# marlbenchmark/off-policy

Measured on NVIDIA H100. Metric: learner grad-steps/sec, higher is better.
Workload: dtype f32

## Files before the change

off-policy_b200/csrc/agent_bwd.cu:

```cuda
#include "mx_internal.h"
#include "mx_kernels.h"
#include "mx_tile.cuh"

static inline size_t qhead_bwd_smem(int A, int APL) { return (size_t)(A * MX_H * 9 + 8 * 32 * APL + 2 * 8 * MX_H + 2 * MX_H) * sizeof(float); }

template <int APL>
__global__ void __launch_bounds__(256) k_qhead_bwd(QHeadBwdArgs a) {
  constexpr int AR = 32 * APL;
  MX_DYN_SMEM(smem);
  const int tid = threadIdx.x, lane = tid & 31, warp = tid >> 5;
  const int A = a.A, AW = A * MX_H;
  float* wq_s = smem;
  float* dw_w = wq_s + AW;
  float* db_w = dw_w + 8 * AW;
  float* dg_w = db_w + 8 * AR;
  float* dbt_w = dg_w + 8 * MX_H;
  float* lg_s = dbt_w + 8 * MX_H;
  float* lb_s = lg_s + MX_H;
  for (int i = tid; i < AW; i += blockDim.x) wq_s[i] = a.theta[a.wq + i];
  for (int i = tid; i < 8 * AW + 8 * AR; i += blockDim.x) dw_w[i] = 0.f;
  for (int i = tid; i < MX_H; i += blockDim.x) { lg_s[i] = a.theta[a.lno_g + i]; lb_s[i] = a.theta[a.lno_b + i]; }
  MX_PDL_WAIT();
  __syncthreads();
  const int wglobal = blockIdx.x * (blockDim.x >> 5) + warp;
  const int wtotal = gridDim.x * (blockDim.x >> 5);
  const int T1 = a.T + 1, N = a.N;
  float dg0 = 0.f, dg1 = 0.f, db0 = 0.f, db1 = 0.f;
  float* my_dw = dw_w + warp * AW;
  for (int m = wglobal; m < a.M; m += wtotal) {
    const int n = m % N;
    const int bt = m / N;
    const int t = bt % T1, b = bt / T1;
    float* out = a.dh_out + (size_t)m * MX_H;
    if (t >= a.T) {
      out[lane] = 0.f; out[lane + 32] = 0.f;
      continue;
    }
    const size_t e = (size_t)b * a.T + t;
    const int act = a.act_idx[(size_t)b * a.ld_tn + (size_t)t * N + n];
    const float dqv = a.dq_taken[e * N + n];
    const float* h = a.hall + (size_t)m * MX_H;
    const float mean = a.sto[2 * (size_t)m], rstd = a.sto[2 * (size_t)m + 1];
    const float xh0 = (h[lane] - mean) * rstd, xh1 = (h[lane + 32] - mean) * rstd;
    const float y0 = xh0 * lg_s[lane] + lb_s[lane], y1 = xh1 * lg_s[lane + 32] + lb_s[lane + 32];
    const float dy0 = dqv * wq_s[act * MX_H + lane], dy1 = dqv * wq_s[act * MX_H + lane + 32];
    my_dw[act * MX_H + lane] += dqv * y0;
    my_dw[act * MX_H + lane + 32] += dqv * y1;
    if (lane == 0) db_w[warp * AR + act] += dqv;
    dg0 += dy0 * xh0; dg1 += dy1 * xh1; db0 += dy0; db1 += dy1;
    const float dx0 = dy0 * lg_s[lane], dx1 = dy1 * lg_s[lane + 32];
    const float c1 = mx_warp_sum(dx0 + dx1) * (1.f / MX_H);
    const float c2 = mx_warp_sum(dx0 * xh0 + dx1 * xh1) * (1.f / MX_H);
    out[lane] = rstd * (dx0 - c1 - xh0 * c2);
    out[lane + 32] = rstd * (dx1 - c1 - xh1 * c2);
  }
  dg_w[warp * MX_H + lane] = dg0; dg_w[warp * MX_H + lane + 32] = dg1;
  dbt_w[warp * MX_H + lane] = db0; dbt_w[warp * MX_H + lane + 32] = db1;
  __syncthreads();
  float* gp = a.gpart + (size_t)blockIdx.x * a.P;
  for (int i = tid; i < AW; i += blockDim.x) {
    float v = 0.f;
#pragma unroll
    for (int w = 0; w < 8; ++w) v += dw_w[w * AW + i];
    gp[a.wq + i] = v;
  }
  for (int i = tid; i < A; i += blockDim.x) {
    float v = 0.f;
#pragma unroll
    for (int w = 0; w < 8; ++w) v += db_w[w * AR + i];
    gp[a.bq + i] = v;
  }
  for (int i = tid; i < MX_H; i += blockDim.x) {
    float g = 0.f, bb = 0.f;
#pragma unroll
    for (int w = 0; w < 8; ++w) { g += dg_w[w * MX_H + i]; bb += dbt_w[w * MX_H + i]; }
    gp[a.lno_g + i] = g; gp[a.lno_b + i] = bb;
  }
}

#define BWD_THREADS 256

template <int RPC>
__global__ void __launch_bounds__(BWD_THREADS, 1) k_gru_bwd(GruBwdArgs a) {
  constexpr int RING = RPC <= 2 ? 8 : 4;
  constexpr int PF = RING - 2;
  __shared__ __align__(16) float ops_s[RING][RPC][6][MX_H];
  __shared__ __align__(16) float dgh_s[2][RPC][MX_G];
  const int tid = threadIdx.x;
  const int k = tid >> 2, s = tid & 3;
  const int row0 = blockIdx.x * RPC;
  float2 w[24];
#pragma unroll
  for (int m = 0; m < 12; ++m)
#pragma unroll
    for (int c = 0; c < 2; ++c) {
      const int j = 16 * m + 4 * s + 2 * c;
      w[2 * m + c] = make_float2(a.theta[a.whh + j * MX_H + k], a.theta[a.whh + (j + 1) * MX_H + k]);
    }
  const int T1 = a.T1 > 0 ? a.T1 : a.T + 1, N = a.N;
  MX_PDL_WAIT();

  constexpr int NPIECE = (RPC * 96 + BWD_THREADS - 1) / BWD_THREADS;
  const float* pf_src[NPIECE];
  size_t pf_stride[NPIECE];
  int pf_dst[NPIECE];
  bool pf_hprev[NPIECE];
  const float* pf_h0[NPIECE];
  const int t_first = a.T - 1;
#pragma unroll
  for (int u = 0; u < NPIECE; ++u) {
    const int c = tid + u * BWD_THREADS;
    pf_dst[u] = -1; pf_src[u] = a.hall; pf_stride[u] = 0; pf_hprev[u] = false; pf_h0[u] = nullptr;
    if (c < RPC * 96) {
      const int r = c / 96, rem = c % 96, op = rem / 16, q4 = rem % 16;
      const int row = row0 + r;
      if (row < a.R) {
        pf_dst[u] = (r * 6 + op) * MX_H + 4 * q4;
        const size_t m0 = ((size_t)(row / N) * T1) * N + (row % N);
        const float* base;
        if (op < 3) { base = a.gates + m0 * MX_G + op * MX_H + 4 * q4; pf_stride[u] = (size_t)N * MX_G; }
        else if (op == 3) { base = a.hn + m0 * MX_H + 4 * q4; pf_stride[u] = (size_t)N * MX_H; }
        else if (op == 4) { base = a.hall + m0 * MX_H + 4 * q4; pf_stride[u] = (size_t)N * MX_H; pf_hprev[u] = true;
                            if (a.h0) pf_h0[u] = a.h0 + (size_t)row * MX_H + 4 * q4; }
        else { base = a.dh_out + m0 * MX_H + 4 * q4; pf_stride[u] = (size_t)N * MX_H; }
        pf_src[u] = base + (ptrdiff_t)(pf_hprev[u] ? t_first - 1 : t_first) * (ptrdiff_t)pf_stride[u];
      }
    }
  }
  auto prefetch = [&](int t) {
    if (t >= 0) {
#pragma unroll
      for (int u = 0; u < NPIECE; ++u) {
        if (pf_dst[u] >= 0) {
          float* dst = &ops_s[t & (RING - 1)][0][0][0] + pf_dst[u];
          const bool first = pf_hprev[u] && t == 0;
          mx_cp16z(dst, first ? (pf_h0[u] ? pf_h0[u] : a.hall) : pf_src[u], (first && !pf_h0[u]) ? 0 : 16);
          pf_src[u] -= pf_stride[u];
        }
      }
    }
    mx_cp_commit();
  };

  for (int idx = tid; idx < RING * RPC * 6 * MX_H; idx += BWD_THREADS) (&ops_s[0][0][0][0])[idx] = 0.f;
  for (int tz = a.T; tz < T1; ++tz)
    for (int idx = tid; idx < RPC * MX_G; idx += BWD_THREADS) {
      const int r = idx / MX_G, c = idx % MX_G;
      const int row = row0 + r;
      if (row < a.R) {
        const size_t mm = (((size_t)(row / N) * T1) + tz) * N + (row % N);
        a.dgi[mm * MX_G + c] = 0.f;
      }
    }
  float* dgp[RPC];
  bool dg_on[RPC];
  float carry[RPC];
  const size_t dg_stride = (size_t)N * MX_G;
  const int sq = s < 3 ? s : 2;
#pragma unroll
  for (int r = 0; r < RPC; ++r) {
    const int row = row0 + r;
    const bool valid = row < a.R;
    const size_t m0 = valid ? ((size_t)(row / N) * T1) * N + (row % N) : 0;
    dgp[r] = a.dgi + (m0 + (size_t)t_first * N) * MX_G + sq * MX_H + k;
    dg_on[r] = valid && s < 3;
    carry[r] = 0.f;
  }
  __syncthreads();
#pragma unroll
  for (int d = 0; d < PF; ++d) prefetch(t_first - d);
  mx_cp_wait<PF - 1>();
  __syncthreads();

  auto step = [&](const int t, const int cur) {
    prefetch(t - PF);
    const float* os = &ops_s[t & (RING - 1)][0][0][0];
    float cz[RPC];
#pragma unroll
    for (int r = 0; r < RPC; ++r) {
      const float* o = os + r * 6 * MX_H;
      const float rg = o[k], zg = o[MX_H + k], ng = o[2 * MX_H + k], hn = o[3 * MX_H + k], hp = o[4 * MX_H + k];
      const float dh = o[5 * MX_H + k] + carry[r];
      const float d_n = dh * (1.f - zg) * (1.f - ng * ng);
      const float d_z = dh * (hp - ng) * zg * (1.f - zg);
      const float d_r = d_n * hn * rg * (1.f - rg);
      const float vg = s == 0 ? d_r : (s == 1 ? d_z : d_n);
      const float vs = s == 0 ? d_r : (s == 1 ? d_z : d_n * rg);
      dgh_s[cur][r][sq * MX_H + k] = vs;
      if (dg_on[r]) *dgp[r] = vg;
      dgp[r] -= dg_stride;
      cz[r] = dh * zg;
    }
    mx_cp_wait<PF - 1>();
    __syncthreads();
#pragma unroll
    for (int r = 0; r < RPC; ++r) {
      float2 p0 = make_float2(0.f, 0.f), p1 = p0, p2 = p0;
#pragma unroll
      for (int m = 0; m < 12; m += 3) {
        const float4 d0 = mx_ld4(&dgh_s[cur][r][16 * m + 4 * s]);
        const float4 d1 = mx_ld4(&dgh_s[cur][r][16 * (m + 1) + 4 * s]);
        const float4 d2 = mx_ld4(&dgh_s[cur][r][16 * (m + 2) + 4 * s]);
        p0 = mx_ffma2(w[2 * m], make_float2(d0.x, d0.y), p0); p0 = mx_ffma2(w[2 * m + 1], make_float2(d0.z, d0.w), p0);
        p1 = mx_ffma2(w[2 * m + 2], make_float2(d1.x, d1.y), p1); p1 = mx_ffma2(w[2 * m + 3], make_float2(d1.z, d1.w), p1);
        p2 = mx_ffma2(w[2 * m + 4], make_float2(d2.x, d2.y), p2); p2 = mx_ffma2(w[2 * m + 5], make_float2(d2.z, d2.w), p2);
      }
      p0 = mx_fadd2(mx_fadd2(p0, p1), p2);
      float p = p0.x + p0.y;
      p += __shfl_xor_sync(0xffffffffu, p, 1);
      p += __shfl_xor_sync(0xffffffffu, p, 2);
      carry[r] = cz[r] + p;
    }
  };
  int t = t_first;
  for (; t >= 1; t -= 2) { step(t, 0); step(t - 1, 1); }
  if (t == 0) step(0, 0);
  mx_cp_wait<0>();
}

#define BWD2_THREADS 128
template <int ROWS>
__global__ void __launch_bounds__(BWD2_THREADS, 2) k_gru_bwd2(GruBwdArgs a) {
  constexpr int RING = 8, PF = 6;
  __shared__ __align__(16) float ops_s[RING][ROWS][6][MX_H];
  __shared__ __align__(16) float dgh_s[2][ROWS][MX_G];
  const int tid = threadIdx.x;
  const int kp = tid >> 2, s = tid & 3;
  float2 w0[24], w1[24];
#pragma unroll
  for (int m = 0; m < 12; ++m)
#pragma unroll
    for (int c = 0; c < 2; ++c) {
      const int j = 16 * m + 4 * s + 2 * c;
      w0[2 * m + c] = make_float2(a.theta[a.whh + j * MX_H + 2 * kp], a.theta[a.whh + (j + 1) * MX_H + 2 * kp]);
      w1[2 * m + c] = make_float2(a.theta[a.whh + j * MX_H + 2 * kp + 1], a.theta[a.whh + (j + 1) * MX_H + 2 * kp + 1]);
    }
  const int T1 = a.T1 > 0 ? a.T1 : a.T + 1, N = a.N;
  MX_PDL_WAIT();
  const int t_first = a.T - 1;
  const bool pf_on = tid < 96;
  const int op = pf_on ? tid / 16 : 0, q4 = tid % 16;
  const bool pf_hprev = op == 4;
  const size_t pf_stride = (size_t)N * (op < 3 ? MX_G : MX_H);
  const int ku = 2 * kp + (s & 1);
  const int half = s >> 1;
  const size_t dg_stride = (size_t)N * MX_G;
  bool rok[ROWS];
  const float* pf_src[ROWS];
  const float* pf_h0[ROWS];
  float* dgp[ROWS];
  float carry[ROWS];
#pragma unroll
  for (int r = 0; r < ROWS; ++r) {
    const int row = blockIdx.x * ROWS + r;
    rok[r] = row < a.R;
    const int rr = rok[r] ? row : 0;
    const size_t m0 = ((size_t)(rr / N) * T1) * N + (rr % N);
    const float* base = op < 3 ? a.gates + m0 * MX_G + op * MX_H + 4 * q4 : (op == 3 ? a.hn : (op == 4 ? a.hall : a.dh_out)) + m0 * MX_H + 4 * q4;
    pf_src[r] = base + (ptrdiff_t)(pf_hprev ? t_first - 1 : t_first) * (ptrdiff_t)pf_stride;
    pf_h0[r] = (pf_hprev && a.h0) ? a.h0 + (size_t)rr * MX_H + 4 * q4 : nullptr;
    if (rok[r])
      for (int tz = a.T; tz < T1; ++tz)
        for (int c = tid; c < MX_G; c += BWD2_THREADS) a.dgi[(m0 + (size_t)tz * N) * MX_G + c] = 0.f;
    dgp[r] = a.dgi + (m0 + (size_t)t_first * N) * MX_G + ku;
    carry[r] = 0.f;
  }
  float* pf_dst = &ops_s[0][0][op][4 * q4];
  auto prefetch = [&](int t) {
    if (t >= 0 && pf_on) {
      const bool first = pf_hprev && t == 0;
#pragma unroll
      for (int r = 0; r < ROWS; ++r) {
        if (rok[r]) mx_cp16z(pf_dst + ((t & (RING - 1)) * ROWS + r) * (6 * MX_H), first ? (pf_h0[r] ? pf_h0[r] : a.hall) : pf_src[r], (first && !pf_h0[r]) ? 0 : 16);
        pf_src[r] -= pf_stride;
      }
    }
    mx_cp_commit();
  };
  if (ROWS > 1) {
    for (int idx = tid; idx < RING * ROWS * 6 * MX_H; idx += BWD2_THREADS) (&ops_s[0][0][0][0])[idx] = 0.f;
    __syncthreads();
  }
#pragma unroll
  for (int d = 0; d < PF; ++d) prefetch(t_first - d);
  mx_cp_wait<PF - 1>();
  __syncthreads();

  auto step = [&](const int t, const int cur) {
    prefetch(t - PF);
    float cz[ROWS];
#pragma unroll
    for (int r = 0; r < ROWS; ++r) {
      const float* o = &ops_s[t & (RING - 1)][r][0][0];
      const float rg = o[ku], zg = o[MX_H + ku], ng = o[2 * MX_H + ku], hn = o[3 * MX_H + ku], hp = o[4 * MX_H + ku];
      const float dh = o[5 * MX_H + ku] + carry[r];
      const float d_n = dh * (1.f - zg) * (1.f - ng * ng);
      const float d_z = dh * (hp - ng) * zg * (1.f - zg);
      const float d_r = d_n * hn * rg * (1.f - rg);
      dgh_s[cur][r][(half ? 2 * MX_H : 0) + ku] = half ? d_n * rg : d_r;
      if (!half) dgh_s[cur][r][MX_H + ku] = d_z;
      if (rok[r]) {
        dgp[r][half ? 2 * MX_H : 0] = half ? d_n : d_r;
        if (!half) dgp[r][MX_H] = d_z;
      }
      dgp[r] -= dg_stride;
      cz[r] = dh * zg;
    }
    mx_cp_wait<PF - 1>();
    __syncthreads();
#pragma unroll
    for (int r = 0; r < ROWS; ++r) {
      float2 a0 = make_float2(0.f, 0.f), a1 = a0, b0 = a0, b1 = a0;
#pragma unroll
      for (int m = 0; m < 12; ++m) {
        const float4 d = mx_ld4(&dgh_s[cur][r][16 * m + 4 * s]);
        const float2 lo = make_float2(d.x, d.y), hi = make_float2(d.z, d.w);
        a0 = mx_ffma2(w0[2 * m], lo, a0); b0 = mx_ffma2(w1[2 * m], lo, b0);
        a1 = mx_ffma2(w0[2 * m + 1], hi, a1); b1 = mx_ffma2(w1[2 * m + 1], hi, b1);
      }
      a0 = mx_fadd2(a0, a1); b0 = mx_fadd2(b0, b1);
      float p0 = a0.x + a0.y, p1 = b0.x + b0.y;
      p0 += __shfl_xor_sync(0xffffffffu, p0, 1); p1 += __shfl_xor_sync(0xffffffffu, p1, 1);
      p0 += __shfl_xor_sync(0xffffffffu, p0, 2); p1 += __shfl_xor_sync(0xffffffffu, p1, 2);
      carry[r] = cz[r] + ((s & 1) ? p1 : p0);
    }
  };
  int t = t_first;
  for (; t >= 1; t -= 2) { step(t, 0); step(t - 1, 1); }
  if (t == 0) step(0, 0);
  mx_cp_wait<0>();
}

struct FrontBwdSmem {
  int ldi, ld64, ldg;
  int o_dgi, o_dgn, o_x, o_hp, o_u, o_da, o_x0, o_xh0, o_dx0, o_wc, o_col, o_stat, o_lnp, total;
};
static FrontBwdSmem front_bwd_smem(int in_dim, int TM, bool gru_ext = false) {
  FrontBwdSmem s;
  const int I64 = mx_round_up(in_dim, 64);
  s.ldi = mx_ld(I64); s.ld64 = mx_ld(64); s.ldg = mx_ld(MX_G);
  int o = 0;
  s.o_dgi = o; o += TM * s.ldg;
  s.o_dgn = o; o += gru_ext ? 0 : TM * s.ld64;
  s.o_x = o; o += TM * s.ld64;
  s.o_hp = o; o += gru_ext ? 0 : TM * s.ld64;
  s.o_u = o; o += TM * s.ld64;
  s.o_da = o; o += TM * s.ld64;
  s.o_x0 = o; o += TM * s.ldi;
  s.o_xh0 = o; o += TM * s.ldi;
  s.o_dx0 = o; o += TM * s.ldi;
  s.o_wc = o; o += 64 * s.ld64;
  s.o_col = o; o += 2 * I64 + 4 * 64;
  s.o_stat = o; o += 3 * TM * 2;
  s.o_lnp = o; o += 4 * 64;
  s.total = o;
  return s;
}

template <int RM>
MX_DEVINL void ln64_bwd_relu(bool act_tanh, float (&v)[RM][4], const float* u_s, int ld, const float* stat , const float* gamma_s,
                             float (&dg)[4], float (&db)[4]) {
  const int tx = threadIdx.x & 15, ty = threadIdx.x >> 4;
#pragma unroll
  for (int i = 0; i < RM; ++i) {
    const int r = ty * RM + i;
    const float mean = stat[2 * r], rstd = stat[2 * r + 1];
    const float4 u4 = mx_ld4(u_s + r * ld + 4 * tx);
    const float uu[4] = {u4.x, u4.y, u4.z, u4.w};
    float xh[4], dx[4], s1 = 0.f, s2 = 0.f;
#pragma unroll
    for (int j = 0; j < 4; ++j) {
      xh[j] = (uu[j] - mean) * rstd;
      dg[j] = fmaf(v[i][j], xh[j], dg[j]);
      db[j] += v[i][j];
      dx[j] = v[i][j] * gamma_s[4 * tx + j];
      s1 += dx[j]; s2 += dx[j] * xh[j];
    }
    s1 = mx_row16_sum(s1) * (1.f / 64.f);
    s2 = mx_row16_sum(s2) * (1.f / 64.f);
#pragma unroll
    for (int j = 0; j < 4; ++j) {
      const float du = rstd * (dx[j] - s1 - xh[j] * s2);
      v[i][j] = act_tanh ? du * (1.f - uu[j] * uu[j]) : (uu[j] > 0.f ? du : 0.f);
    }
  }
}

template <int RM>
__global__ void __launch_bounds__(MX_TILE_THREADS) k_front_bwd(FrontBwdArgs a, FrontBwdSmem sm) {
  constexpr int TM = 16 * RM;
  MX_DYN_SMEM(smem);
  const MxNetLayout L = a.L;
  const float* __restrict__ th = a.theta;
  const int I = L.in_dim, I64 = mx_round_up(I, 64);
  float* dgi_s = smem + sm.o_dgi; float* dgn_s = smem + sm.o_dgn; float* x_s = smem + sm.o_x; float* hp_s = smem + sm.o_hp;
  float* u_s = smem + sm.o_u; float* da_s = smem + sm.o_da; float* x0_s = smem + sm.o_x0; float* xh0_s = smem + sm.o_xh0;
  float* Wc = smem + sm.o_wc;
  float* col0g = smem + sm.o_col; float* col0b = col0g + I64;
  float* col1g = col0b + I64; float* col1b = col1g + 64;
  float* col2g = col1b + 64; float* col2b = col2g + 64;
  float* st0_s = smem + sm.o_stat; float* st1_s = st0_s + 2 * TM; float* st2_s = st1_s + 2 * TM;
  float* ln1g_s = smem + sm.o_lnp; float* ln1b_s = ln1g_s + 64; float* ln2g_s = ln1b_s + 64; float* ln2b_s = ln2g_s + 64;
  const int tid = threadIdx.x, tx = tid & 15, ty = tid >> 4;
  const int ntiles = (a.M + TM - 1) / TM;
  const int T1 = a.T1 > 0 ? a.T1 : a.T + 1, N = a.N;
  const bool ldx_vec = (a.ldx & 3) == 0;
  const bool wg = !a.skip_wgrad;
  const bool wgemm = wg && !a.wgrad_external;
  const bool gru_here = !a.gru_wgrad_ext;
  float* dx0_s = smem + sm.o_dx0;
  float* gp = a.gpart + (size_t)blockIdx.x * a.P;
  for (int i = tid; i < 2 * I64 + 4 * 64; i += MX_TILE_THREADS) col0g[i] = 0.f;
  if (tid < 64) { ln1g_s[tid] = th[L.ln1_g + tid]; ln1b_s[tid] = th[L.ln1_b + tid]; ln2g_s[tid] = th[L.ln2_g + tid]; ln2b_s[tid] = th[L.ln2_b + tid]; }
  float dg1[4] = {0.f, 0.f, 0.f, 0.f}, db1[4] = {0.f, 0.f, 0.f, 0.f}, dg2[4] = {0.f, 0.f, 0.f, 0.f}, db2[4] = {0.f, 0.f, 0.f, 0.f};
  int iter = 0;
  MX_PDL_WAIT();
  for (int tile = blockIdx.x; tile < ntiles; tile += gridDim.x, ++iter) {
    const int m0 = tile * TM;
    const bool accum = iter > 0;
    __syncthreads();
    mx_stage_rows(dgi_s, sm.ldg, a.dgi, MX_G, m0, a.M, TM, MX_G);
    if (!gru_here) {}
    else if (!a.no_gru) mx_stage_rows(x_s, sm.ld64, a.gates, MX_G, m0, a.M, TM, MX_H);
    else for (int i = tid; i < TM * sm.ld64; i += MX_TILE_THREADS) x_s[i] = 0.f;
    mx_stage_rows(u_s, sm.ld64, a.u2, MX_H, m0, a.M, TM, MX_H);
    for (int r = tid >> 4; gru_here && r < TM; r += MX_TILE_THREADS / 16) {
      const int m = m0 + r;
      const bool has = !a.no_gru && m < a.M && ((m / N) % T1) > 0;
      float* d = hp_s + r * sm.ld64 + 4 * tx;
      if (has) mx_cp16(d, a.hall + (size_t)(m - N) * MX_H + 4 * tx);
      else if (m < a.M && a.h0) mx_cp16(d, a.h0 + (size_t)m * MX_H + 4 * tx);
      else mx_st4(d, make_float4(0.f, 0.f, 0.f, 0.f));
    }
    if (ldx_vec) mx_stage_rows(x0_s, sm.ldi, a.X, a.ldx, m0, a.M, TM, mx_round_up(I, 4));
    mx_cp_commit();
    for (int i = tid; i < 3 * TM * 2; i += MX_TILE_THREADS) {
      const int which = i / (2 * TM), rr = (i % (2 * TM)) >> 1, comp = i & 1;
      const int m = m0 + rr;
      const float* src = which == 0 ? a.st0 : (which == 1 ? a.st1 : a.st2);
      st0_s[i] = (m < a.M && (which > 0 || a.feature_norm)) ? src[2 * (size_t)m + comp] : 0.f;
    }
    mx_cp_wait<0>();
    __syncthreads();
    for (int idx = tid; gru_here && idx < TM * MX_H; idx += MX_TILE_THREADS) {
      const int r = idx >> 6, c = idx & 63;
      const int o = r * sm.ld64 + c;
      dgn_s[o] = dgi_s[r * sm.ldg + 2 * MX_H + c] * x_s[o];
      x_s[o] = (m0 + r < a.M) ? (u_s[o] - st2_s[2 * r]) * st2_s[2 * r + 1] * ln2g_s[c] + ln2b_s[c] : 0.f;
    }
    __syncthreads();
    if (wgemm && gru_here) {
      for (int nb = 0; nb < 3; ++nb) {
        mx_wgrad_block(dgi_s + nb * 64, sm.ldg, x_s, sm.ld64, TM, gp + L.wih, MX_G, MX_H, nb * 64, 0, accum);
        if (a.no_gru) continue;
        const float* dgh = nb < 2 ? dgi_s + nb * 64 : dgn_s;
        const int ldd = nb < 2 ? sm.ldg : sm.ld64;
        mx_wgrad_block(dgh, ldd, hp_s, sm.ld64, TM, gp + L.whh + nb * 64 * MX_H, 64, MX_H, 0, 0, accum);
      }
      mx_colsum(dgi_s, sm.ldg, TM, MX_G, gp + L.bih, accum);
      if (!a.no_gru) {
        mx_colsum(dgi_s, sm.ldg, TM, 2 * MX_H, gp + L.bhh, accum);
        mx_colsum(dgn_s, sm.ld64, TM, MX_H, gp + L.bhh + 2 * MX_H, accum);
      }
    }
    float v[RM][4];
#pragma unroll
    for (int i = 0; i < RM; ++i)
#pragma unroll
      for (int jx = 0; jx < 4; ++jx) v[i][jx] = 0.f;
    for (int nc = 0; nc < 3; ++nc) {
      __syncthreads();
      mx_stage_weight(Wc, sm.ld64, th + L.wih, MX_G, MX_H, MX_H, nc * 64, 0, 64);
      __syncthreads();
      mx_mm_nn<RM>(dgi_s + nc * 64, sm.ldg, Wc, sm.ld64, v);
    }
    ln64_bwd_relu<RM>(a.act_tanh != 0, v, u_s, sm.ld64, st2_s, ln2g_s, dg2, db2);
    __syncthreads();
#pragma unroll
    for (int i = 0; i < RM; ++i) mx_st4(da_s + (ty * RM + i) * sm.ld64 + 4 * tx, make_float4(v[i][0], v[i][1], v[i][2], v[i][3]));
    if (a.wgrad_external) {
#pragma unroll
      for (int i = 0; i < RM; ++i) {
        const int m = m0 + ty * RM + i;
        if (m < a.M) mx_st4(a.da2_out + (size_t)m * MX_H + 4 * tx, make_float4(v[i][0], v[i][1], v[i][2], v[i][3]));
      }
    }
    mx_stage_rows(u_s, sm.ld64, a.u1, MX_H, m0, a.M, TM, MX_H);
    mx_cp_commit();
    mx_cp_wait<0>();
    __syncthreads();
    for (int idx = tid; idx < TM * MX_H; idx += MX_TILE_THREADS) {
      const int r = idx >> 6, c = idx & 63;
      const int o = r * sm.ld64 + c;
      x_s[o] = (m0 + r < a.M) ? (u_s[o] - st1_s[2 * r]) * st1_s[2 * r + 1] * ln1g_s[c] + ln1b_s[c] : 0.f;
    }
    __syncthreads();
    if (wgemm) {
      mx_wgrad_block(da_s, sm.ld64, x_s, sm.ld64, TM, gp + L.w2, MX_H, MX_H, 0, 0, accum);
      mx_colsum(da_s, sm.ld64, TM, MX_H, gp + L.b2, accum);
    }
    mx_stage_weight(Wc, sm.ld64, th + L.w2, MX_H, MX_H, MX_H, 0, 0, 64);
    __syncthreads();
#pragma unroll
    for (int i = 0; i < RM; ++i)
#pragma unroll
      for (int jx = 0; jx < 4; ++jx) v[i][jx] = 0.f;
    mx_mm_nn<RM>(da_s, sm.ld64, Wc, sm.ld64, v);
    ln64_bwd_relu<RM>(a.act_tanh != 0, v, u_s, sm.ld64, st1_s, ln1g_s, dg1, db1);
    __syncthreads();
#pragma unroll
    for (int i = 0; i < RM; ++i) mx_st4(da_s + (ty * RM + i) * sm.ld64 + 4 * tx, make_float4(v[i][0], v[i][1], v[i][2], v[i][3]));
    if (a.wgrad_external) {
#pragma unroll
      for (int i = 0; i < RM; ++i) {
        const int m = m0 + ty * RM + i;
        if (m < a.M) mx_st4(a.da1_out + (size_t)m * MX_H + 4 * tx, make_float4(v[i][0], v[i][1], v[i][2], v[i][3]));
      }
    }
    for (int idx = tid; idx < TM * I64; idx += MX_TILE_THREADS) {
      const int r = idx / I64, c = idx - r * I64, m = m0 + r;
      float xh = 0.f, x0 = 0.f;
      if (m < a.M && c < I) {
        const float x = ldx_vec ? x0_s[r * sm.ldi + c] : a.X[(size_t)m * a.ldx + c];
        if (a.feature_norm) {
          xh = (x - st0_s[2 * r]) * st0_s[2 * r + 1];
          x0 = xh * th[L.fn_g + c] + th[L.fn_b + c];
        } else x0 = x;
      }
      x0_s[r * sm.ldi + c] = x0; xh0_s[r * sm.ldi + c] = xh;
    }
    __syncthreads();
    if (wgemm) {
      for (int kb = 0; kb * 64 < I; ++kb) {
        mx_wgrad_block(da_s, sm.ld64, x0_s + kb * 64, sm.ldi, TM, gp + L.w1, MX_H, I, 0, kb * 64, accum);
      }
      mx_colsum(da_s, sm.ld64, TM, MX_H, gp + L.b1, accum);
    }
    if (a.feature_norm || a.dX) {
      for (int kb = 0; kb * 64 < I; ++kb) {
        __syncthreads();
        mx_stage_weight(Wc, sm.ld64, th + L.w1, MX_H, I, I, 0, kb * 64, 64);
        __syncthreads();
#pragma unroll
        for (int i = 0; i < RM; ++i)
#pragma unroll
          for (int jx = 0; jx < 4; ++jx) v[i][jx] = 0.f;
        mx_mm_nn<RM>(da_s, sm.ld64, Wc, sm.ld64, v);
        float cg[4] = {0.f, 0.f, 0.f, 0.f}, cb[4] = {0.f, 0.f, 0.f, 0.f};
#pragma unroll
        for (int jx = 0; jx < 4; ++jx) {
          const int c = kb * 64 + 4 * tx + jx;
          if (c < I) {
            float sg = 0.f, sb = 0.f;
#pragma unroll
            for (int i = 0; i < RM; ++i) {
              sg = fmaf(v[i][jx], xh0_s[(ty * RM + i) * sm.ldi + c], sg); sb += v[i][jx];
              if (a.dX) dx0_s[(ty * RM + i) * sm.ldi + c] = v[i][jx];
            }
            cg[jx] = sg; cb[jx] = sb;
          }
        }
        if (wg && a.feature_norm) {
          for (int g = 0; g < MX_TILE_THREADS / 16; ++g) {
            if (ty == g) {
#pragma unroll
              for (int jx = 0; jx < 4; ++jx) {
                const int c = kb * 64 + 4 * tx + jx;
                if (c < I) { col0g[c] += cg[jx]; col0b[c] += cb[jx]; }
              }
            }
            __syncthreads();
          }
        }
      }
      if (a.dX) {
        __syncthreads();
        const int lane = tid & 31, warp = tid >> 5;
        for (int r = warp; r < TM; r += MX_TILE_THREADS / 32) {
          const int m = m0 + r;
          if (m >= a.M) continue;
          float s1 = 0.f, s2 = 0.f;
          for (int c = lane; c < I; c += 32) {
            const float dxh = dx0_s[r * sm.ldi + c] * (a.feature_norm ? th[L.fn_g + c] : 1.f);
            s1 += dxh; s2 += dxh * xh0_s[r * sm.ldi + c];
          }
          s1 = mx_warp_sum(s1) / (float)I; s2 = mx_warp_sum(s2) / (float)I;
          const float rstd = st0_s[2 * r + 1];
          for (int c = lane; c < I; c += 32) {
            const float d0 = dx0_s[r * sm.ldi + c];
            a.dX[(size_t)m * a.ldx + c] = a.feature_norm ? rstd * (d0 * th[L.fn_g + c] - s1 - xh0_s[r * sm.ldi + c] * s2) : d0;
          }
        }
      }
    }
  }
  for (int g = 0; g < MX_TILE_THREADS / 16; ++g) {
    if (ty == g) {
#pragma unroll
      for (int jx = 0; jx < 4; ++jx) {
        const int c = 4 * tx + jx;
        col1g[c] += dg1[jx]; col1b[c] += db1[jx];
        col2g[c] += dg2[jx]; col2b[c] += db2[jx];
      }
    }
    __syncthreads();
  }
  if (wg) {
    for (int c = tid; c < MX_H; c += MX_TILE_THREADS) {
      gp[L.ln2_g + c] = col2g[c]; gp[L.ln2_b + c] = col2b[c];
      gp[L.ln1_g + c] = col1g[c]; gp[L.ln1_b + c] = col1b[c];
    }
    for (int c = tid; c < I; c += MX_TILE_THREADS) { gp[L.fn_g + c] = col0g[c]; gp[L.fn_b + c] = col0b[c]; }
  }
}


struct GruWgradSmem { int ld64, ldg, o_dgi, o_dgn, o_x, o_hp, o_stat, o_lnp, total; };
static GruWgradSmem gru_wgrad_smem(int TM) {
// ... 211 lines not shown
```

off-policy_b200/csrc/agent_fwd.cu:

```cuda
#include "mx_internal.h"
#include "mx_kernels.h"
#include "mx_tile.cuh"

template <int RM>
__global__ void __launch_bounds__(MX_TILE_THREADS) k_front_fwd(FrontFwdArgs a) {
  constexpr int TM = 16 * RM;
  MX_DYN_SMEM(smem);
  const int net = blockIdx.y;
  const float* __restrict__ th = a.theta[net];
  const MxNetLayout L = a.L;
  const int I = L.in_dim, Ipad = (I + 3) & ~3;
  const int lda = mx_ld_dev(Ipad > MX_H ? Ipad : MX_H);
  const int ldw = lda;
  float* A_s = smem;
  float* Wc = A_s + TM * lda;
  const int tid = threadIdx.x, tx = tid & 15, ty = tid >> 4, lane = tid & 31, warp = tid >> 5;
  const bool live = (net == 0);
  const int ntiles = (a.M + TM - 1) / TM;
  MX_PDL_WAIT();

  for (int tile = blockIdx.x; tile < ntiles; tile += gridDim.x) {
    const int m0 = tile * TM;
    if (I <= 128) {
      constexpr int RW = TM / (MX_TILE_THREADS / 32);
      float xv[RW][4];
#pragma unroll
      for (int q = 0; q < RW; ++q) {
        const int m = m0 + warp + q * (MX_TILE_THREADS / 32);
#pragma unroll
        for (int u = 0; u < 4; ++u) {
          const int c = lane + 32 * u;
          xv[q][u] = (m < a.M && c < I) ? a.X[(size_t)m * a.ldx + c] : 0.f;
        }
      }
#pragma unroll
      for (int q = 0; q < RW; ++q) {
        const int r = warp + q * (MX_TILE_THREADS / 32), m = m0 + r;
        float* row = A_s + r * lda;
        const float mean = mx_warp_sum(xv[q][0] + xv[q][1] + xv[q][2] + xv[q][3]) / (float)I;
        float qq = 0.f;
#pragma unroll
        for (int u = 0; u < 4; ++u) { const float d = (lane + 32 * u < I) ? xv[q][u] - mean : 0.f; qq += d * d; }
        const float rstd = rsqrtf(mx_warp_sum(qq) / (float)I + MX_LN_EPS);
#pragma unroll
        for (int u = 0; u < 4; ++u) {
          const int c = lane + 32 * u;
          if (c < Ipad) {
            float v = 0.f;
            if (c < I && m < a.M) v = a.feature_norm ? ((xv[q][u] - mean) * rstd * th[L.fn_g + c] + th[L.fn_b + c]) : xv[q][u];
            row[c] = v;
          }
        }
        if (live && lane == 0 && a.st0 && m < a.M) { a.st0[2 * (size_t)m] = mean; a.st0[2 * (size_t)m + 1] = rstd; }
      }
    } else
    for (int r = warp; r < TM; r += MX_TILE_THREADS / 32) {
      const int m = m0 + r;
      float* row = A_s + r * lda;
      if (m < a.M) {
        const float* x = a.X + (size_t)m * a.ldx;
        float s = 0.f;
        for (int c = lane; c < I; c += 32) s += x[c];
        const float mean = mx_warp_sum(s) / (float)I;
        float q = 0.f;
        for (int c = lane; c < I; c += 32) { float d = x[c] - mean; q += d * d; }
        const float rstd = rsqrtf(mx_warp_sum(q) / (float)I + MX_LN_EPS);
        for (int c = lane; c < Ipad; c += 32) {
          float v = 0.f;
          if (c < I) v = a.feature_norm ? ((x[c] - mean) * rstd * th[L.fn_g + c] + th[L.fn_b + c]) : x[c];
          row[c] = v;
        }
        if (live && lane == 0 && a.st0) { a.st0[2 * (size_t)m] = mean; a.st0[2 * (size_t)m + 1] = rstd; }
      } else {
        for (int c = lane; c < Ipad; c += 32) row[c] = 0.f;
      }
    }
    for (int layer = 0; layer < 2; ++layer) {
      const int K = layer == 0 ? I : MX_H, Kpad = (K + 3) & ~3;
      const int w_off = layer == 0 ? L.w1 : L.w2, b_off = layer == 0 ? L.b1 : L.b2;
      const int g_off = layer == 0 ? L.ln1_g : L.ln2_g, be_off = layer == 0 ? L.ln1_b : L.ln2_b;
      mx_stage_weight(Wc, ldw, th + w_off, MX_H, K, K, 0, 0, Kpad);
      __syncthreads();
      float acc[RM][4];
#pragma unroll
      for (int i = 0; i < RM; ++i)
#pragma unroll
        for (int j = 0; j < 4; ++j) acc[i][j] = 0.f;
      mx_mm_nt<RM>(A_s, lda, Wc, ldw, Kpad, acc);
#pragma unroll
      for (int i = 0; i < RM; ++i)
#pragma unroll
        for (int j = 0; j < 4; ++j) { const float z = acc[i][j] + th[b_off + tx + 16 * j]; acc[i][j] = a.act_tanh ? tanhf(z) : fmaxf(z, 0.f); }
      float mean[RM], rstd[RM];
      mx_row_stats64<RM>(acc, mean, rstd);
      float* u_out = layer == 0 ? a.u1 : a.u2;
      float* st_out = layer == 0 ? a.st1 : a.st2;
      __syncthreads();
#pragma unroll
      for (int i = 0; i < RM; ++i) {
        const int r = ty * RM + i, m = m0 + r;
#pragma unroll
        for (int j = 0; j < 4; ++j) {
          const int c = tx + 16 * j;
          A_s[r * lda + c] = (acc[i][j] - mean[i]) * rstd[i] * th[g_off + c] + th[be_off + c];
          if (live && m < a.M && u_out) u_out[(size_t)m * MX_H + c] = acc[i][j];
        }
        if (live && m < a.M && tx == 0 && st_out) { st_out[2 * (size_t)m] = mean[i]; st_out[2 * (size_t)m + 1] = rstd[i]; }
      }
    }
    float* gi = a.gi[net];
    for (int c3 = 0; c3 < 3; ++c3) {
      mx_stage_weight(Wc, ldw, th + L.wih, MX_G, MX_H, MX_H, 64 * c3, 0, MX_H);
      __syncthreads();
      float acc[RM][4];
#pragma unroll
      for (int i = 0; i < RM; ++i)
#pragma unroll
        for (int j = 0; j < 4; ++j) acc[i][j] = 0.f;
      mx_mm_nt<RM>(A_s, lda, Wc, ldw, MX_H, acc);
#pragma unroll
      for (int i = 0; i < RM; ++i) {
        const int m = m0 + ty * RM + i;
        if (m < a.M) {
#pragma unroll
          for (int j = 0; j < 4; ++j) {
            const int c = 64 * c3 + tx + 16 * j;
            gi[(size_t)m * MX_G + c] = acc[i][j] + th[L.bih + c];
          }
        }
      }
      __syncthreads();
    }
  }
}

#define GRU_PF 5
#define GRU_RING 8
#define GRU_THREADS 256

template <int RPC>
__global__ void __launch_bounds__(GRU_THREADS, 1) k_gru_fwd(GruFwdArgs a) {
  __shared__ __align__(16) float h_s[2][RPC][MX_H];
  __shared__ __align__(16) float gi_s[GRU_RING][RPC][MX_G];
  const int net = blockIdx.y;
  const float* __restrict__ th = a.theta[net];
  const int tid = threadIdx.x;
  const int i = tid >> 2, q = tid & 3;
  const int row0 = blockIdx.x * RPC;
  const bool live = (net == 0) && a.gates != nullptr;
  float2 wr[8], wz[8], wn[8];
#pragma unroll
  for (int m = 0; m < 4; ++m)
#pragma unroll
    for (int c = 0; c < 2; ++c) {
      const int k = 16 * m + 4 * q + 2 * c;
      wr[2 * m + c] = make_float2(th[a.whh + i * MX_H + k], th[a.whh + i * MX_H + k + 1]);
      wz[2 * m + c] = make_float2(th[a.whh + (MX_H + i) * MX_H + k], th[a.whh + (MX_H + i) * MX_H + k + 1]);
      wn[2 * m + c] = make_float2(th[a.whh + (2 * MX_H + i) * MX_H + k], th[a.whh + (2 * MX_H + i) * MX_H + k + 1]);
    }
  const float br = th[a.bhh + i], bz = th[a.bhh + MX_H + i], bn = th[a.bhh + 2 * MX_H + i];
  MX_PDL_WAIT();
  for (int idx = tid; idx < 2 * RPC * MX_H; idx += GRU_THREADS) {
    const int r = (idx / MX_H) % RPC, c = idx % MX_H;
    (&h_s[0][0][0])[idx] = (a.h0 && row0 + r < a.R) ? a.h0[(size_t)(row0 + r) * MX_H + c] : 0.f;
  }
  for (int idx = tid; idx < GRU_RING * RPC * MX_G; idx += GRU_THREADS) (&gi_s[0][0][0])[idx] = 0.f;

  const float* gi = a.gi[net];
  const int T1 = a.T + 1, N = a.N;
  float* stp[RPC];
  float* hnp[RPC];
  bool st_on[RPC], hn_on[RPC];
  const size_t st_stride = (size_t)N * (q == 0 ? MX_H : MX_G), hn_stride = (size_t)N * MX_H;
#pragma unroll
  for (int r = 0; r < RPC; ++r) {
    const int row = row0 + r;
    const bool valid = row < a.R;
    const int b = valid ? row / N : 0, n = valid ? row % N : 0;
    const size_t m0 = ((size_t)b * T1) * N + n;
    stp[r] = (q == 0) ? a.hall[net] + m0 * MX_H + i : (live ? a.gates + m0 * MX_G + (q - 1) * MX_H + i : nullptr);
    hnp[r] = live ? a.hn + m0 * MX_H + i : nullptr;
    st_on[r] = valid && (q == 0 || live);
    hn_on[r] = valid && live && q == 0;
  }
  const int pf_r = tid / (MX_G / 4), pf_q = tid % (MX_G / 4);
  const bool pf_on = tid < RPC * (MX_G / 4) && (row0 + pf_r) < a.R;
  const float* pf_src = gi;
  float* pf_dst = &gi_s[0][0][0];
  if (pf_on) {
    const int row = row0 + pf_r;
    pf_src = gi + (((size_t)(row / N) * T1) * N + (row % N)) * MX_G + 4 * pf_q;
    pf_dst = &gi_s[0][pf_r][4 * pf_q];
  }
  const size_t pf_stride = (size_t)N * MX_G;
  auto prefetch = [&](int t) {
    if (pf_on && t < T1) { mx_cp16(pf_dst + (t & (GRU_RING - 1)) * (RPC * MX_G), pf_src); pf_src += pf_stride; }
    mx_cp_commit();
  };
  __syncthreads();
#pragma unroll
  for (int t = 0; t < GRU_PF; ++t) prefetch(t);
  mx_cp_wait<GRU_PF - 1>();
  __syncthreads();

  auto step = [&](const int t, const int cur) {
    const int nxt = cur ^ 1;
    prefetch(t + GRU_PF);
    const float* gs = &gi_s[t & (GRU_RING - 1)][0][0];
#pragma unroll
    for (int r = 0; r < RPC; ++r) {
      const float* hrow = &h_s[cur][r][0];
      const float* g = gs + r * MX_G;
      float4 hv[4];
#pragma unroll
      for (int m = 0; m < 4; ++m) hv[m] = mx_ld4(hrow + 16 * m + 4 * q);
      const float gr = g[i] + br, gz = g[MX_H + i] + bz, gn = g[2 * MX_H + i], hp = hrow[i];
      float2 r0 = make_float2(0.f, 0.f), r1 = r0, z0 = r0, z1 = r0, n0 = r0, n1 = r0;
#pragma unroll
      for (int m = 0; m < 4; ++m) {
        const float2 lo = make_float2(hv[m].x, hv[m].y), hi = make_float2(hv[m].z, hv[m].w);
        r0 = mx_ffma2(wr[2 * m], lo, r0); z0 = mx_ffma2(wz[2 * m], lo, z0); n0 = mx_ffma2(wn[2 * m], lo, n0);
        r1 = mx_ffma2(wr[2 * m + 1], hi, r1); z1 = mx_ffma2(wz[2 * m + 1], hi, z1); n1 = mx_ffma2(wn[2 * m + 1], hi, n1);
      }
      r0 = mx_fadd2(r0, r1); z0 = mx_fadd2(z0, z1); n0 = mx_fadd2(n0, n1);
      float pr = r0.x + r0.y, pz = z0.x + z0.y, pn = n0.x + n0.y;
      pr += __shfl_xor_sync(0xffffffffu, pr, 1); pn += __shfl_xor_sync(0xffffffffu, pn, 1); pz += __shfl_xor_sync(0xffffffffu, pz, 1);
      pr += __shfl_xor_sync(0xffffffffu, pr, 2); pn += __shfl_xor_sync(0xffffffffu, pn, 2); pz += __shfl_xor_sync(0xffffffffu, pz, 2);
      const float rg = mx_sigmoid_fast(pr + gr);
      const float hn = pn + bn;
      const float ng = mx_tanh_fast(fmaf(rg, hn, gn));
      const float zg = mx_sigmoid_fast(pz + gz);
      const float hnew = fmaf(zg, hp - ng, ng);
      h_s[nxt][r][i] = hnew;
      const float v = q == 0 ? hnew : (q == 1 ? rg : (q == 2 ? zg : ng));
      if (st_on[r]) *stp[r] = v;
      if (hn_on[r]) *hnp[r] = hn;
      stp[r] += st_stride; hnp[r] += hn_stride;
    }
    mx_cp_wait<GRU_PF - 1>();
    __syncthreads();
  };
  int t = 0;
  for (; t + 1 < T1; t += 2) { step(t, 0); step(t + 1, 1); }
  if (t < T1) step(t, 0);
  mx_cp_wait<0>();
}

#define GRU2_THREADS 128
template <int ROWS>
__global__ void __launch_bounds__(GRU2_THREADS, 2) k_gru_fwd2(GruFwdArgs a) {
  __shared__ __align__(16) float h_s[2][ROWS][MX_H];
  __shared__ __align__(16) float gi_s[GRU_RING][ROWS][MX_G];
  const int net = blockIdx.y;
  const float* __restrict__ th = net ? a.theta[1] : a.theta[0];
  const int tid = threadIdx.x;
  const int i = tid >> 1, q = tid & 1;
  const bool live = (net == 0) && a.gates != nullptr;
  float2 wr[16], wz[16], wn[16];
#pragma unroll
  for (int m = 0; m < 8; ++m)
#pragma unroll
    for (int c = 0; c < 2; ++c) {
      const int k = 8 * m + 4 * q + 2 * c;
      wr[2 * m + c] = make_float2(th[a.whh + i * MX_H + k], th[a.whh + i * MX_H + k + 1]);
      wz[2 * m + c] = make_float2(th[a.whh + (MX_H + i) * MX_H + k], th[a.whh + (MX_H + i) * MX_H + k + 1]);
      wn[2 * m + c] = make_float2(th[a.whh + (2 * MX_H + i) * MX_H + k], th[a.whh + (2 * MX_H + i) * MX_H + k + 1]);
    }
  const float br = th[a.bhh + i], bz = th[a.bhh + MX_H + i], bn = th[a.bhh + 2 * MX_H + i];
  MX_PDL_WAIT();
  const float* gi = net ? a.gi[1] : a.gi[0];
  float* hall = net ? a.hall[1] : a.hall[0];
  const int T1 = a.T + 1, N = a.N;
  float *p1[ROWS], *p2[ROWS], *p3[ROWS];
  bool rok[ROWS];
  const float* pf_src[ROWS];
  const bool pf_on = tid < MX_G / 4;
#pragma unroll
  for (int r = 0; r < ROWS; ++r) {
    const int row = blockIdx.x * ROWS + r;
    rok[r] = row < a.R;
    const int rr = rok[r] ? row : 0;
    for (int idx = tid; idx < 2 * MX_H; idx += GRU2_THREADS) (&h_s[0][0][0])[(idx >> 6) * ROWS * MX_H + r * MX_H + (idx & 63)] = (a.h0 && idx < MX_H && rok[r]) ? a.h0[(size_t)rr * MX_H + idx] : 0.f;
    const int b = rr / N, n = rr % N;
    const size_t m0 = ((size_t)b * T1) * N + n;
    p1[r] = q == 0 ? hall + m0 * MX_H + i : (live ? a.gates + m0 * MX_G + MX_H + i : hall);
    p2[r] = live ? a.gates + m0 * MX_G + (q == 0 ? 0 : 2 * MX_H) + i : hall;
    p3[r] = live ? a.hn + m0 * MX_H + i : hall;
    pf_src[r] = gi + m0 * MX_G + 4 * (pf_on ? tid : 0);
  }
  const bool on1 = q == 0 || live, on2 = live, on3 = live && q == 0;
  const size_t s1 = (size_t)N * ((q == 0) ? MX_H : MX_G), s2 = (size_t)N * MX_G, s3 = (size_t)N * MX_H;
  float* pf_dst = &gi_s[0][0][4 * (pf_on ? tid : 0)];
  const size_t pf_stride = (size_t)N * MX_G;
  auto prefetch = [&](int t) {
    if (pf_on && t < T1) {
#pragma unroll
      for (int r = 0; r < ROWS; ++r) {
        if (rok[r]) mx_cp16(pf_dst + ((t & (GRU_RING - 1)) * ROWS + r) * MX_G, pf_src[r]);
        pf_src[r] += pf_stride;
      }
    }
    mx_cp_commit();
  };
#pragma unroll
  for (int t = 0; t < GRU_PF; ++t) prefetch(t);
  mx_cp_wait<GRU_PF - 1>();
  __syncthreads();

  auto step = [&](const int t, const int cur) {
    const int nxt = cur ^ 1;
    prefetch(t + GRU_PF);
#pragma unroll
    for (int r = 0; r < ROWS; ++r) {
      const float* g = &gi_s[t & (GRU_RING - 1)][r][0];
      const float* hrow = &h_s[cur][r][0];
      float4 hv[8];
#pragma unroll
      for (int m = 0; m < 8; ++m) hv[m] = mx_ld4(hrow + 8 * m + 4 * q);
      const float gr = g[i] + br, gz = g[MX_H + i] + bz, gn = g[2 * MX_H + i], hp = hrow[i];
      float2 r0 = make_float2(0.f, 0.f), r1 = r0, z0 = r0, z1 = r0, n0 = r0, n1 = r0;
#pragma unroll
      for (int m = 0; m < 8; ++m) {
        const float2 lo = make_float2(hv[m].x, hv[m].y), hi = make_float2(hv[m].z, hv[m].w);
        r0 = mx_ffma2(wr[2 * m], lo, r0); n0 = mx_ffma2(wn[2 * m], lo, n0); z0 = mx_ffma2(wz[2 * m], lo, z0);
        r1 = mx_ffma2(wr[2 * m + 1], hi, r1); n1 = mx_ffma2(wn[2 * m + 1], hi, n1); z1 = mx_ffma2(wz[2 * m + 1], hi, z1);
      }
      r0 = mx_fadd2(r0, r1); n0 = mx_fadd2(n0, n1); z0 = mx_fadd2(z0, z1);
      float pr = r0.x + r0.y, pn = n0.x + n0.y, pz = z0.x + z0.y;
      pr += __shfl_xor_sync(0xffffffffu, pr, 1); pn += __shfl_xor_sync(0xffffffffu, pn, 1); pz += __shfl_xor_sync(0xffffffffu, pz, 1);
      const float rg = mx_sigmoid_fast(pr + gr);
      const float hn = pn + bn;
      const float ng = mx_tanh_fast(fmaf(rg, hn, gn));
      const float zg = mx_sigmoid_fast(pz + gz);
      const float hnew = fmaf(zg, hp - ng, ng);
      h_s[nxt][r][i] = hnew;
      if (rok[r]) {
        if (on1) *p1[r] = q == 0 ? hnew : zg;
        if (on2) *p2[r] = q == 0 ? rg : ng;
        if (on3) *p3[r] = hn;
      }
      p1[r] += s1; p2[r] += s2; p3[r] += s3;
    }
    mx_cp_wait<GRU_PF - 1>();
    __syncthreads();
  };
  int t = 0;
  for (; t + 1 < T1; t += 2) { step(t, 0); step(t + 1, 1); }
  if (t < T1) step(t, 0);
  mx_cp_wait<0>();
}

template <int APL>
__global__ void __launch_bounds__(256) k_qhead(QHeadArgs a) {
  __shared__ float wq_s[2][32 * APL * MX_H];
  __shared__ float bq_s[2][32 * APL];
  __shared__ float lg_s[2][MX_H], lb_s[2][MX_H];
  const int tid = threadIdx.x, lane = tid & 31;
  const int A = a.A;
  for (int net = 0; net < 2; ++net) {
    const float* th = a.theta[net];
    for (int i = tid; i < A * MX_H; i += blockDim.x) wq_s[net][i] = th[a.wq + i];
    for (int i = tid; i < A; i += blockDim.x) bq_s[net][i] = th[a.bq + i];
    for (int i = tid; i < MX_H; i += blockDim.x) { lg_s[net][i] = th[a.lno_g + i]; lb_s[net][i] = th[a.lno_b + i]; }
  }
  MX_PDL_WAIT();
  __syncthreads();
  const int wglobal = blockIdx.x * (blockDim.x >> 5) + (tid >> 5);
  const int wtotal = gridDim.x * (blockDim.x >> 5);
  const int T1 = a.T + 1, N = a.N;
  for (int m = wglobal; m < a.M; m += wtotal) {
    const int n = m % N;
    const int bt = m / N;
    const int t = bt % T1, b = bt / T1;
    float q_live_at_act = 0.f, tq_sel = 0.f;
    int greedy = 0;
    const float* hl = a.hall[0] + (size_t)m * MX_H;
    const float* ht = a.hall[1] + (size_t)m * MX_H;
    const float hl0 = hl[lane], hl1 = hl[lane + 32], ht0 = ht[lane], ht1 = ht[lane + 32];
    const int act = (t < a.T) ? a.act_idx[(size_t)b * a.ld_tn + (size_t)t * N + n] : 0;
    float av = 1.f;
    if (a.avail && lane < A) av = a.avail[(size_t)m * a.act_ld + lane];
    const unsigned avail_mask = __ballot_sync(0xffffffffu, av != 0.f);
    unsigned avail_hi = 0u;
    if constexpr (APL == 2) {
      float av2 = 1.f;
      if (a.avail && lane + 32 < A) av2 = a.avail[(size_t)m * a.act_ld + lane + 32];
      avail_hi = __ballot_sync(0xffffffffu, av2 != 0.f);
    }
    {
      const float mean = mx_warp_sum(hl0 + hl1) * (1.f / MX_H);
      const float d0 = hl0 - mean, d1 = hl1 - mean;
      const float rstd = rsqrtf(mx_warp_sum(d0 * d0 + d1 * d1) * (1.f / MX_H) + MX_LN_EPS);
      if (lane == 0) { a.sto[2 * (size_t)m] = mean; a.sto[2 * (size_t)m + 1] = rstd; }
      const float y0 = d0 * rstd * lg_s[0][lane] + lb_s[0][lane];
      const float y1 = d1 * rstd * lg_s[0][lane + 32] + lb_s[0][lane + 32];
      float best = 0.f;
      for (int k = 0; k < A; ++k) {
        float q = mx_warp_sum(y0 * wq_s[0][k * MX_H + lane] + y1 * wq_s[0][k * MX_H + lane + 32]) + bq_s[0][k];
        if (a.qall0 && lane == 0) a.qall0[(size_t)m * A + k] = q;
        if (k == act) q_live_at_act = q;
        unsigned on;
        if constexpr (APL == 1) on = (avail_mask >> k) & 1u;
        else on = ((k < 32 ? avail_mask : avail_hi) >> (k & 31)) & 1u;
        const float qm = on ? q : -1e10f;
        if (k == 0 || qm > best) { best = qm; greedy = k; }
      }
    }
    {
      const float mean = mx_warp_sum(ht0 + ht1) * (1.f / MX_H);
      const float d0 = ht0 - mean, d1 = ht1 - mean;
      const float rstd = rsqrtf(mx_warp_sum(d0 * d0 + d1 * d1) * (1.f / MX_H) + MX_LN_EPS);
      const float y0 = d0 * rstd * lg_s[1][lane] + lb_s[1][lane];
      const float y1 = d1 * rstd * lg_s[1][lane + 32] + lb_s[1][lane + 32];
      float tbest = 0.f;
      for (int k = 0; k < A; ++k) {
        float q = mx_warp_sum(y0 * wq_s[1][k * MX_H + lane] + y1 * wq_s[1][k * MX_H + lane + 32]) + bq_s[1][k];
        if (a.qall1 && lane == 0) a.qall1[(size_t)m * A + k] = q;
        if (a.double_q) { if (k == greedy) tq_sel = q; }
        else if (k == 0 || q > tbest) { tbest = q; tq_sel = q; }
      }
    }
    if (lane == 0) {
      if (a.greedy) a.greedy[m] = greedy;
      if (t < a.T) a.q_taken[((size_t)b * a.T + t) * N + n] = q_live_at_act;
      if (t >= 1) a.q_next[((size_t)b * a.T + (t - 1)) * N + n] = tq_sel;
    }
  }
}

__global__ void __launch_bounds__(256) k_mlp_qselect(MlpQSelArgs a) {
  const int total = a.B * a.N;
  MX_PDL_WAIT();
  for (int i = blockIdx.x * blockDim.x + threadIdx.x; i < total; i += gridDim.x * blockDim.x) {
    const int n = i % a.N, b = i / a.N;
    const size_t m0 = ((size_t)b * 2) * a.N + n, m1 = m0 + a.N;
    const float* q0 = a.gi[0] + m0 * MX_G;
    const float* q1 = a.gi[0] + m1 * MX_G;
    const float* t1 = a.gi[1] + m1 * MX_G;
    const int act = a.act_idx[(size_t)b * a.ld_tn + n];
    int greedy = 0;
    float best = 0.f, tbest = 0.f;
    for (int k = 0; k < a.A; ++k) {
      const bool off = a.avail && a.avail[m1 * a.act_ld + k] == 0.f;
      const float qm = off ? -1e10f : q1[k];
      if (k == 0 || qm > best) { best = qm; greedy = k; }
      const float tm = off ? -1e10f : t1[k];
      if (k == 0 || tm > tbest) tbest = tm;
    }
    a.q_taken[i] = q0[act];
    a.q_next[i] = a.double_q ? t1[greedy] : tbest;
    if (a.greedy) { a.greedy[m0] = 0; a.greedy[m1] = greedy; }
    if (a.qall0)
      for (int k = 0; k < a.A; ++k) {
        a.qall0[m0 * a.A + k] = q0[k]; a.qall0[m1 * a.A + k] = q1[k];
        a.qall1[m0 * a.A + k] = a.gi[1][m0 * MX_G + k]; a.qall1[m1 * a.A + k] = t1[k];
      }
  }
}
int mx_launch_mlp_qselect(const MlpQSelArgs& a, cudaStream_t s) {
  int grid = mx_ceil_div(a.B * a.N, 256);
  if (grid > mx_num_sms() * 4) grid = mx_num_sms() * 4;
  return mx_launch("k_mlp_qselect", k_mlp_qselect, dim3(grid), dim3(256), 0, s, MX_STEP, a);
}

__global__ void __launch_bounds__(256) k_pack_prev_act(const float* __restrict__ obs, int obs_ld, const float* __restrict__ acts, int act_ld,
                                                       float* __restrict__ X, int ldx, int B, int T, int N, int O, int A) {
  const long long total = (long long)B * (T + 1) * N * ldx;
  MX_PDL_WAIT();
  for (long long i = (long long)blockIdx.x * blockDim.x + threadIdx.x; i < total; i += (long long)gridDim.x * blockDim.x) {
    const int c = (int)(i % ldx);
    const long long m = i / ldx;
    const int n = (int)(m % N);
    const long long bt = m / N;
    const int t = (int)(bt % (T + 1));
    const long long b = bt / (T + 1);
    float v = 0.f;
    if (c < O) v = obs[m * obs_ld + c];
    else if (c < O + A && t > 0) v = acts[((b * T + (t - 1)) * N + n) * act_ld + (c - O)];
    X[i] = v;
  }
}

int mx_launch_pack_prev_act(const float* obs, int obs_ld, const float* acts, int act_ld, float* X, int ldx, int B, int T, int N, int O, int A,
                            cudaStream_t s) {
  const long long total = (long long)B * (T + 1) * N * ldx;
  int grid = (int)((total + 255) / 256);
  const int cap = mx_num_sms() * 8;
  if (grid > cap) grid = cap;
  return mx_launch("k_pack_prev_act", k_pack_prev_act, dim3(grid), dim3(256), 0, s, MX_STEP, obs, obs_ld, acts, act_ld, X, ldx, B, T, N, O, A);
}

size_t mx_front_fwd_smem(int in_dim, int RM) {
  const int Ipad = mx_round_up(in_dim, 4);
  const int lda = mx_ld(Ipad > MX_H ? Ipad : MX_H);
  return (size_t)(16 * RM + 64) * lda * sizeof(float);
}

extern int g_mx_front_tc;
int mx_launch_front_fwd_tc(const FrontFwdArgs& a, int nets, cudaStream_t s);
bool mx_front_tc_usable(int in_dim, bool have_image);

int mx_launch_front_fwd(const FrontFwdArgs& a, int nets, cudaStream_t s) {
  if (mx_front_tc_usable(a.L.in_dim, a.tc_img[0] != nullptr) && (a.ldx & 3) == 0) return mx_launch_front_fwd_tc(a, nets, s);
  const int RM = 2;
  const int ntiles = mx_ceil_div(a.M, 16 * RM);
  int gx = mx_num_sms() / nets;
  if (gx < 1) gx = 1;
  if (gx > ntiles) gx = ntiles;
  const size_t smem = mx_front_fwd_smem(a.L.in_dim, RM);
  return mx_launch("k_front_fwd", k_front_fwd<RM>, dim3(gx, nets), dim3(MX_TILE_THREADS), smem, s, MX_STEP, a);
}

int mx_launch_gru_fwd(const GruFwdArgs& a, int nets, cudaStream_t s) {
  const int sms = mx_num_sms();
  int rpc = 1;
  while (rpc < 4 && mx_ceil_div(a.R, rpc) * nets > 2 * sms) rpc *= 2;
  if (a.T + 1 >= 8) return mx_launch("k_gru_fwd", k_gru_fwd2<1>, dim3(a.R, nets), dim3(GRU2_THREADS), 0, s, MX_STEP, a);
  auto kern = rpc == 1 ? k_gru_fwd<1> : rpc == 2 ? k_gru_fwd<2> : k_gru_fwd<4>;
  return mx_launch("k_gru_fwd", kern, dim3(mx_ceil_div(a.R, rpc), nets), dim3(GRU_THREADS), 0, s, MX_STEP, a);
}

int mx_launch_qhead(const QHeadArgs& a, cudaStream_t s) {
  if (a.A > 64) { mx_set_error("qhead: act_dim %d > 64 unsupported", a.A); return 1; }
  int grid = mx_ceil_div(a.M, 8);
  const int cap = mx_num_sms() * 4;
  if (grid > cap) grid = cap;
  return mx_launch("k_qhead", a.A > 32 ? k_qhead<2> : k_qhead<1>, dim3(grid), dim3(256), 0, s, MX_STEP, a);
}
```

Measured before the change: 4663.

## Reorder GRU recurrence steps to hoist shared loads and defer global stores

In the forward GRU scan, the per-step shared-memory loads of the hidden state and gate inputs are hoisted ahead of the cp.async prefetch. The global stores of hnew, gates and hn are deferred by one step so they overlap with the next step's matvec. In the backward scan, the shared dgh values are loaded into registers before the next prefetch is issued and before the global gradient stores. The cp.async wait depth is relaxed to PF-2. The goal is to take global-store and async-copy issue latency off the serial recurrence critical path, at the cost of higher register pressure and a shallower effective prefetch distance.

```diff
diff --git a/off-policy_b200/csrc/agent_bwd.cu b/off-policy_b200/csrc/agent_bwd.cu
--- a/off-policy_b200/csrc/agent_bwd.cu
+++ b/off-policy_b200/csrc/agent_bwd.cu
@@ -287,8 +287,7 @@
   __syncthreads();
 
   auto step = [&](const int t, const int cur) {
-    prefetch(t - PF);
-    float cz[ROWS];
+    float cz[ROWS], vr[ROWS], vz[ROWS];
 #pragma unroll
     for (int r = 0; r < ROWS; ++r) {
       const float* o = &ops_s[t & (RING - 1)][r][0][0];
@@ -299,21 +298,31 @@
       const float d_r = d_n * hn * rg * (1.f - rg);
       dgh_s[cur][r][(half ? 2 * MX_H : 0) + ku] = half ? d_n * rg : d_r;
       if (!half) dgh_s[cur][r][MX_H + ku] = d_z;
+      vr[r] = half ? d_n : d_r; vz[r] = d_z;
+      cz[r] = dh * zg;
+    }
+    mx_cp_wait<PF - 2>();
+    __syncthreads();
+    float4 dv[ROWS][12];
+#pragma unroll
+    for (int r = 0; r < ROWS; ++r)
+#pragma unroll
+      for (int m = 0; m < 12; ++m) dv[r][m] = mx_ld4(&dgh_s[cur][r][16 * m + 4 * s]);
+    prefetch(t - PF);
+#pragma unroll
+    for (int r = 0; r < ROWS; ++r) {
       if (rok[r]) {
-        dgp[r][half ? 2 * MX_H : 0] = half ? d_n : d_r;
-        if (!half) dgp[r][MX_H] = d_z;
+        dgp[r][half ? 2 * MX_H : 0] = vr[r];
+        if (!half) dgp[r][MX_H] = vz[r];
       }
       dgp[r] -= dg_stride;
-      cz[r] = dh * zg;
-    }
-    mx_cp_wait<PF - 1>();
-    __syncthreads();
+    }
 #pragma unroll
     for (int r = 0; r < ROWS; ++r) {
       float2 a0 = make_float2(0.f, 0.f), a1 = a0, b0 = a0, b1 = a0;
 #pragma unroll
       for (int m = 0; m < 12; ++m) {
-        const float4 d = mx_ld4(&dgh_s[cur][r][16 * m + 4 * s]);
+        const float4 d = dv[r][m];
         const float2 lo = make_float2(d.x, d.y), hi = make_float2(d.z, d.w);
         a0 = mx_ffma2(w0[2 * m], lo, a0); b0 = mx_ffma2(w1[2 * m], lo, b0);
         a1 = mx_ffma2(w0[2 * m + 1], hi, a1); b1 = mx_ffma2(w1[2 * m + 1], hi, b1);
diff --git a/off-policy_b200/csrc/agent_fwd.cu b/off-policy_b200/csrc/agent_fwd.cu
--- a/off-policy_b200/csrc/agent_fwd.cu
+++ b/off-policy_b200/csrc/agent_fwd.cu
@@ -307,39 +307,51 @@
   mx_cp_wait<GRU_PF - 1>();
   __syncthreads();
 
+  float sv1[ROWS], sv2[ROWS], shn[ROWS];
+  auto store = [&]() {
+#pragma unroll
+    for (int r = 0; r < ROWS; ++r) {
+      if (rok[r]) {
+        if (on1) *p1[r] = sv1[r];
+        if (on2) *p2[r] = sv2[r];
+        if (on3) *p3[r] = shn[r];
+      }
+      p1[r] += s1; p2[r] += s2; p3[r] += s3;
+    }
+  };
   auto step = [&](const int t, const int cur) {
     const int nxt = cur ^ 1;
-    prefetch(t + GRU_PF);
+    float4 hv[ROWS][8];
+    float gr[ROWS], gz[ROWS], gn[ROWS], hp[ROWS];
 #pragma unroll
     for (int r = 0; r < ROWS; ++r) {
       const float* g = &gi_s[t & (GRU_RING - 1)][r][0];
       const float* hrow = &h_s[cur][r][0];
-      float4 hv[8];
-#pragma unroll
-      for (int m = 0; m < 8; ++m) hv[m] = mx_ld4(hrow + 8 * m + 4 * q);
-      const float gr = g[i] + br, gz = g[MX_H + i] + bz, gn = g[2 * MX_H + i], hp = hrow[i];
+#pragma unroll
+      for (int m = 0; m < 8; ++m) hv[r][m] = mx_ld4(hrow + 8 * m + 4 * q);
+      gr[r] = g[i] + br; gz[r] = g[MX_H + i] + bz; gn[r] = g[2 * MX_H + i]; hp[r] = hrow[i];
+    }
+    prefetch(t + GRU_PF);
+    if (t > 0) store();
+#pragma unroll
+    for (int r = 0; r < ROWS; ++r) {
       float2 r0 = make_float2(0.f, 0.f), r1 = r0, z0 = r0, z1 = r0, n0 = r0, n1 = r0;
 #pragma unroll
       for (int m = 0; m < 8; ++m) {
-        const float2 lo = make_float2(hv[m].x, hv[m].y), hi = make_float2(hv[m].z, hv[m].w);
+        const float2 lo = make_float2(hv[r][m].x, hv[r][m].y), hi = make_float2(hv[r][m].z, hv[r][m].w);
         r0 = mx_ffma2(wr[2 * m], lo, r0); n0 = mx_ffma2(wn[2 * m], lo, n0); z0 = mx_ffma2(wz[2 * m], lo, z0);
         r1 = mx_ffma2(wr[2 * m + 1], hi, r1); n1 = mx_ffma2(wn[2 * m + 1], hi, n1); z1 = mx_ffma2(wz[2 * m + 1], hi, z1);
       }
       r0 = mx_fadd2(r0, r1); n0 = mx_fadd2(n0, n1); z0 = mx_fadd2(z0, z1);
       float pr = r0.x + r0.y, pn = n0.x + n0.y, pz = z0.x + z0.y;
       pr += __shfl_xor_sync(0xffffffffu, pr, 1); pn += __shfl_xor_sync(0xffffffffu, pn, 1); pz += __shfl_xor_sync(0xffffffffu, pz, 1);
-      const float rg = mx_sigmoid_fast(pr + gr);
+      const float rg = mx_sigmoid_fast(pr + gr[r]);
       const float hn = pn + bn;
-      const float ng = mx_tanh_fast(fmaf(rg, hn, gn));
-      const float zg = mx_sigmoid_fast(pz + gz);
-      const float hnew = fmaf(zg, hp - ng, ng);
+      const float ng = mx_tanh_fast(fmaf(rg, hn, gn[r]));
+      const float zg = mx_sigmoid_fast(pz + gz[r]);
+      const float hnew = fmaf(zg, hp[r] - ng, ng);
       h_s[nxt][r][i] = hnew;
-      if (rok[r]) {
-        if (on1) *p1[r] = q == 0 ? hnew : zg;
-        if (on2) *p2[r] = q == 0 ? rg : ng;
-        if (on3) *p3[r] = hn;
-      }
-      p1[r] += s1; p2[r] += s2; p3[r] += s3;
+      sv1[r] = q == 0 ? hnew : zg; sv2[r] = q == 0 ? rg : ng; shn[r] = hn;
     }
     mx_cp_wait<GRU_PF - 1>();
     __syncthreads();
@@ -347,6 +359,7 @@
   int t = 0;
   for (; t + 1 < T1; t += 2) { step(t, 0); step(t + 1, 1); }
   if (t < T1) step(t, 0);
+  store();
   mx_cp_wait<0>();
 }
 
```

Result: slower. 4502 (median of 6 runs) (-3.5%).
